# emiliofidalgo/liodom

Hardware: AMD Instinct MI355X
Metric: scans/sec (64×1800 cloud, prev_frames=20) at 1 GPU; pose RMSE vs CPU ref (higher is better)
Workload: dtype f64

## Files before the change

### liodom_amd/csrc/kernels_lm.h

```cpp
__host__ __device__ __forceinline__ bool lm_lds_reduce_fits(int edge_cap) {
  return (size_t)((edge_cap + 3) & ~3) * sizeof(int) + (size_t)kAccN * kLmEvalThreads * sizeof(double) + 8192 <= 160 * 1024;
}
__host__ __device__ __forceinline__ size_t lm_lds_bytes(int edge_cap) {
  return (size_t)((edge_cap + 3) & ~3) * sizeof(int) +
         (lm_lds_reduce_fits(edge_cap) ? (size_t)kAccN * kLmEvalThreads : (size_t)(kLmThreads / 16) * kAccN) * sizeof(double);
}


__device__ int lm_compact_bits(const DevView& v, int s, int outer_it, int E, int* idx ) {
  const int lane = threadIdx.x & 63;
  const int Q = v.knn_queries;
  const int nb = (E + Q - 1) / Q;
  const int nwords = (nb + 3) >> 2;
  const unsigned int* mw = reinterpret_cast<const unsigned int*>(v.corr_mask + ((size_t)s * 2 + outer_it) * v.mask_stride);
  int run = 0;
  for (int w0 = 0; w0 < nwords; w0 += 64) {
    const int w = w0 + lane;
    unsigned int word = (w < nwords) ? mw[w] : 0u;
    const int pop = __popc(word);
    const int incl = wave_incl_scan_i32(pop);
    int o = run + incl - pop;
    while (word) {
      const int b = __ffs(word) - 1;
      word &= word - 1u;
// ... 8 lines not shown
#ifndef LIODOM_LM_CACHED
#define LIODOM_LM_CACHED 1
#endif
constexpr int kLmCached = LIODOM_LM_CACHED;
struct LmCache { float4 P[kLmCached], A[kLmCached], B[kLmCached]; };
__device__ __forceinline__ void lm_cache_load(const DevView& v, int s, int outer_it, int eb, int c_lo, int c_hi, const int* idx, LmCache& k) {
  const float4* ed = v.edges + ((size_t)eb * v.n_streams + s) * v.edge_cap;
  const float4* ca = v.corr_a + ((size_t)s * 2 + outer_it) * v.edge_cap;
  const float4* cb = v.corr_b + ((size_t)s * 2 + outer_it) * v.edge_cap;
  const int et = (int)threadIdx.x;
#pragma unroll
  for (int j = 0; j < kLmCached; j++) {
    const int c = c_lo + et + j * kLmEvalThreads;
    if (et < kLmCtl && c < c_hi) { const int e = idx[c]; k.A[j] = ca[e]; k.B[j] = cb[e]; k.P[j] = ed[e]; }
  }
}

__device__ __forceinline__ void lm_eval(const DevView& v, int s, int outer_it, int eb, int c_lo, int c_hi, const int* idx, const double* Rm_sh,
                                        double* part, double* acc_out , const LmCache& k) {
  const int et = (int)threadIdx.x;
#ifdef LIODOM_LM_NOCACHE
  const bool cached = false;
#else
  const bool cached = et < kLmCtl;
#endif
  double acc[kAccN];
#pragma unroll
  for (int i = 0; i < kAccN; i++) acc[i] = 0.0;
  {
    double Rm[12];
#pragma unroll
    for (int i = 0; i < 12; i++) Rm[i] = Rm_sh[i];
    const float4* ed = v.edges + ((size_t)eb * v.n_streams + s) * v.edge_cap;
    const float4* ca = v.corr_a + ((size_t)s * 2 + outer_it) * v.edge_cap;
    const float4* cb = v.corr_b + ((size_t)s * 2 + outer_it) * v.edge_cap;
    int c = c_lo + et;
    if (cached) {
#pragma unroll
      for (int j = 0; j < kLmCached; j++, c += kLmEvalThreads) {
        if (c < c_hi) {
          const double p[3] = {(double)k.P[j].x, (double)k.P[j].y, (double)k.P[j].z};
          const double a[3] = {(double)k.A[j].x, (double)k.A[j].y, (double)k.A[j].z};
          const double b[3] = {(double)k.B[j].x, (double)k.B[j].y, (double)k.B[j].z};
          residual_accumulate(Rm, p, a, b, v.min_range, v.max_range, acc);
        }
      }
    }
    for (; c < c_hi; c += kLmEvalThreads) {
      const int e = idx[c];
      const float4 A = ca[e];
      const float4 B = cb[e];
      const float4 P = ed[e];
      const double p[3] = {(double)P.x, (double)P.y, (double)P.z};
      const double a[3] = {(double)A.x, (double)A.y, (double)A.z};
      const double b[3] = {(double)B.x, (double)B.y, (double)B.z};
      residual_accumulate(Rm, p, a, b, v.min_range, v.max_range, acc);
    }
  }
  if (v.lm_lds_reduce) {
    const int nb_here = c_hi - c_lo;
    const int ncol = ((nb_here < kLmEvalThreads ? nb_here : kLmEvalThreads) + 15) & ~15;
    if (et < ncol) {
#pragma unroll
      for (int i = 0; i < kAccN; i++) part[i * kLmEvalThreads + et] = acc[i];
    }
    __syncthreads();
    const int r = threadIdx.x & 15;
#pragma unroll
    for (int vrow = threadIdx.x >> 4; vrow < ((kAccN + kLmThreads / 16 - 1) / (kLmThreads / 16)) * (kLmThreads / 16); vrow += kLmThreads / 16) {
      double x = 0.0;
      if (vrow < kAccN) {
        const double* rowp = part + vrow * kLmEvalThreads + r;
        const int nk = ncol >> 4;
#pragma unroll 8
        for (int kk = 0; kk < nk; kk++) x += rowp[kk * 16];
      }
      x = row_sum_f64(x);
      if (vrow < kAccN && r == 0) acc_out[vrow] = x;
    }
    __syncthreads();
    return;
  }
#pragma unroll
  for (int i = 0; i < kAccN; i++) acc[i] = row_sum_f64(acc[i]);
  const int row = threadIdx.x >> 4;
  if ((threadIdx.x & 15) == 0) {
#pragma unroll
    for (int i = 0; i < kAccN; i++) part[row * kAccN + i] = acc[i];
  }
  __syncthreads();
  if (threadIdx.x < kAccN) {
    double x = 0.0;
    for (int w = 0; w < kLmThreads / 16; w++) x += part[w * kAccN + threadIdx.x];
    acc_out[threadIdx.x] = x;
  }
  __syncthreads();
}

__device__ void hash_clear_used(const DevView& v, int s , int nup, int t, int nt) {
  CellSlot empty; empty.key = kEmptyKey; empty.start = 0; empty.cnt = 0;
  const int* used = v.used_cells + (size_t)s * v.used_cap;
  if (nup > v.used_cap) nup = v.used_cap;
  for (int u0 = t; u0 < nup; u0 += 8 * nt) {
    int hh[8];
#pragma unroll
    for (int k = 0; k < 8; k++) { const int u = u0 + k * nt; hh[k] = (u < nup) ? used[u] : -1; }
#pragma unroll
    for (int k = 0; k < 8; k++) {
      if (hh[k] >= 0) {
        const size_t ti = (size_t)s * v.table_size + hh[k];
        v.cells[ti] = empty;
        v.cell_bits[ti >> 5] = 0u;
        if (v.cell_pad) v.cell_pad[ti] = 0u;
      }
    }
  }
}
// ... 159 lines not shown
  if (!st.initialized) return;
  double odom[12], out[12], l2b[12], q[4];
#pragma unroll
  for (int k = 0; k < 12; k++) { odom[k] = st.odom[k]; l2b[k] = v.laser_to_base[k]; }
#pragma unroll
  for (int k = 0; k < 4; k++) q[k] = v.imu_q[(size_t)(s0 + i) * 4 + k];
  imu_override(odom, q, l2b, v.rotation_mode, out);
#pragma unroll
  for (int k = 0; k < 12; k++) st.odom[k] = out[k];
  quat_from_pose(out, v.rotation_mode, st.param_q);
  st.param_t[0] = out[3]; st.param_t[1] = out[7]; st.param_t[2] = out[11];
}

__device__ __forceinline__ void rebuild_beside_solve(const DevView& v, int s, StreamState& st, int eb, int outer_it, int block, int nblocks, unsigned int seq, int* sbase, int* sslot);

template <int kOuterIt, bool kChainMode>
#ifndef LIODOM_LM_WAVES_PER_SIMD
#define LIODOM_LM_WAVES_PER_SIMD 1
#endif
__global__ __launch_bounds__(kLmThreads, LIODOM_LM_WAVES_PER_SIMD) void k_lm_solve(DevView v, int s0, int eb, unsigned int seq, unsigned int done_target) {
  constexpr int outer_it = kOuterIt;
  constexpr int chain = kChainMode ? 1 : 0;
  __shared__ double sh_pose2[2][12];
  __shared__ int sh_pi, sh_ci;
  __shared__ int sh_nmoved;
  __shared__ double sh_pred_s[20];
  __shared__ int sh_unapplied;
  __shared__ double sh_acc[kAccN];
  __shared__ LmState lm;
  __shared__ int sh_flag;
  __shared__ int sh_C;
  const int s = s0 + blockIdx.y;
#if defined(LIODOM_CHAIN_PRIO)
  if (v.n_streams <= 4) __builtin_amdgcn_s_setprio(LIODOM_CHAIN_PRIO);
#endif
  const int G = v.lm_groups, gstride = G > 1 ? 8 : 1, bxl = (int)blockIdx.x;
  const bool is_solver = bxl < G * gstride && (bxl % gstride) == 0;
  const int g = is_solver ? bxl / gstride : G + (bxl < G * gstride ? bxl - (bxl / gstride + 1) : bxl - G);
  StreamState& st = v.state[s];
  __shared__ int sh_cnt[kMaxFrames + 1];
  __shared__ int sh_same_xcc;
  OV_STAMP(v, bxl == 0 && threadIdx.x == 0, outer_it == 0 ? 0 : 3);
  if (seq && outer_it == 0 && bxl == 0 && threadIdx.x == 0) {
    typedef __attribute__((address_space(1))) unsigned int gu32;
    __hip_atomic_store((gu32*)(v.ov_flags + s), seq, __ATOMIC_RELAXED, __HIP_MEMORY_SCOPE_AGENT);
  }
  if (g >= G) {
    if (!v.early_rebuild || chain) return;
    __shared__ int sh_slot[kMaxFrames];
    rebuild_beside_solve(v, s, st, eb, outer_it, g - G, (int)gridDim.x - G, seq, sh_cnt, sh_slot);
    return;
  }
  __shared__ double sh_loc[kAccN];
  __shared__ double sh_red[16][32];
  __shared__ double sh_x0[8];
  __shared__ double sh_prev[12];
  __shared__ int sh_fc;
  if (threadIdx.x < 4) sh_x0[threadIdx.x] = st.param_q[threadIdx.x];
  else if (threadIdx.x < 7) sh_x0[threadIdx.x] = st.param_t[threadIdx.x - 4];
  else if (threadIdx.x >= 64 && threadIdx.x < 76) sh_prev[threadIdx.x - 64] = st.prev_odom[threadIdx.x - 64];
  else if (threadIdx.x == 76) sh_fc = st.frame_count;
  __shared__ int sh_spec_at;
  if (threadIdx.x == 77) sh_spec_at = st.spec_eval[outer_it];
  __shared__ int sh_redo;
  if (threadIdx.x == 78) sh_redo = st.spec_redo[outer_it == 0 ? 1 : 0];
  extern __shared__ __attribute__((aligned(16))) int sh_idx[];
  double* sh_part = reinterpret_cast<double*>(sh_idx + ((v.edge_cap + 3) & ~3));
  const int tid = threadIdx.x;
  const bool prep = tid < kLmCtl;
  bool dead = false;
  if (chain && outer_it == 0) dead = !chain_wait_count(v.knn_done0 + s, done_target, &st.status);
  if (chain && outer_it == 0 && sh_redo) __builtin_amdgcn_fence(__ATOMIC_ACQUIRE, "agent");
  int E_in;
  if (chain && outer_it == 0) {
    typedef __attribute__((address_space(1))) unsigned int gu32;
    E_in = (int)__hip_atomic_load((gu32*)(v.edge_cnt + eb * 32 + s), __ATOMIC_RELAXED, __HIP_MEMORY_SCOPE_AGENT);
  } else {
    E_in = st.n_edges_buf[eb];
  }
  if (outer_it == 0 && tid == 0 && g == 0) {
    st.info.n_edges = E_in;
    st.info.map_points = st.n_search;
    for (int k = 0; k < 2; k++) {
      st.info.lm[k].iterations = 0; st.info.lm[k].accepted = 0; st.info.lm[k].termination = LM_TERM_NO_RESIDUALS;
      st.info.lm[k].pad = 0; st.info.lm[k].initial_cost = 0.0; st.info.lm[k].final_cost = 0.0;
    }
  }
  if (!st.initialized) {
    if (outer_it == 1 && g == 0) {
      if (seq) ov_wait_knn_done(v, s, seq, &st.status);
      if (tid == 0) st.append_raw = 1;
      __shared__ double sh_T0[12];
// ... 49 lines not shown
        for (int u = 0; u < 16; u += 2) { x0 += xs[u]; x1 += xs[u + 1]; }
      }
    }
    sh_red[r0][i] = x0 + x1;
    __syncthreads();
    if (tid <= kAccN) {
      double x = 0.0;
#pragma unroll
      for (int r = 0; r < kRC; r++) x += sh_red[r][tid];
      if (tid < kAccN) sh_acc[tid] = x;
      else { sh_nmatch = (int)x; if (g == 0) st.info.matches[outer_it] = (int)x; }
    }
    __syncthreads();
    nblocks = sh_nmatch;
  } else {
    __syncthreads();
    if (prep) {
      const int C = lm_compact_bits(v, s, outer_it, E, sh_idx);
      if (tid == 0) sh_C = C;
    } else if (tid == kLmCtl) {
      iso_from_qt(sh_x0, sh_x0 + 4, sh_pose2[0]);
    }
    __syncthreads();
    my_share(sh_C);
    lm_cache_load(v, s, outer_it, eb, c_lo, c_hi, sh_idx, cache);
    if (G > 1) { lm_eval(v, s, outer_it, eb, c_lo, c_hi, sh_idx, sh_pose2[0], sh_part, sh_loc, cache); lm_exchange(v, s, g, G, epoch0 | ++n_eval, sh_loc, sh_acc, &st.status, xch_local, &sh_same_xcc); xch_local = sh_same_xcc != 0; }
    else { lm_eval(v, s, outer_it, eb, c_lo, c_hi, sh_idx, sh_pose2[0], sh_part, sh_acc, cache); ++n_eval; }
  }
  DBG_STAMP(v, dbgb, 2, 2);
  int dbg_it = 0;
  int pi = 0, ci = -1, nmoved = 0;
  const unsigned int n_eval0 = n_eval;
  const bool spec_ok = v.speculate != 0 && v.speculate != 5 && v.speculate != 7 && g == 0 && seq != 0u && outer_it == 0;
  const bool spec_ok1 = v.speculate != 0 && v.speculate != 4 && v.speculate != 6 && g == 0 && chain != 0 && outer_it == 1 && v.early_rebuild && v.pred_xch != nullptr;
  const bool spec_forced = v.speculate == 2 || v.speculate == 6 || v.speculate == 7;
  bool spec_done = false;
  int spec_moves = -1;
  for (int step = 0;; step++) {
    if (step == 0 && tid > kLmCtl && tid <= kLmCtl + 6) {
      const int j = tid - kLmCtl - 1;
      sh_scale[j] = 1.0 / (1.0 + sqrt(sh_acc[7 + h_idx(j, j)]));
    }
    if (step == 0) __builtin_amdgcn_wave_barrier();
    if (tid == kLmCtl) {
      const int acc_before = step == 0 ? 0 : lm.accepted;
      const int f = step == 0 ? lm_begin(lm, sh_x0, sh_x0 + 4, sh_acc, nblocks, v.apply_on_ftol, sh_scale) : lm_update(lm, sh_acc);
      sh_flag = f;
      bool moved = step > 0 && lm.accepted != acc_before;
      if (step > 0 && !moved && f != LM_NEED_EVAL && lm.termination == LM_TERM_FUNC_TOL) {
        moved = true;
        for (int k = 0; k < 4; k++) moved = moved && lm.q[k] == lm.cand_q[k];
        for (int k = 0; k < 3; k++) moved = moved && lm.t[k] == lm.cand_t[k];
      }
      if (moved) { ci = pi; pi ^= 1; nmoved++; }
      if (f == LM_NEED_EVAL) iso_from_qt(lm.cand_q, lm.cand_t, sh_pose2[pi]);
      sh_pi = pi; sh_ci = ci; sh_nmoved = nmoved; sh_unapplied = (step > 0 && !moved) ? 1 : 0;
      if (step == 0) DBG_STAMP(v, dbgb, 2, 23);
    } else if (!prep) {
    } else if (step == 0 && v.knn_partials) {
      DBG_STAMP(v, dbge, 2, 24);
      const int C = dead ? 0 : lm_compact_bits(v, s, outer_it, E, sh_idx);
      if (tid == 0) sh_C = C;
      DBG_STAMP(v, dbge, 2, 25);
      my_share(C);
      lm_cache_load(v, s, outer_it, eb, c_lo, c_hi, sh_idx, cache);
    } else if (clr_pending) {
      clear_hash_slots();
    }
    __syncthreads();
    if (step == 0) { if (v.knn_partials && !prep) my_share(sh_C); DBG_STAMP(v, dbgb, 2, 3); }
    else { DBG_STAMP(v, dbgb && dbg_it < 5, 2, 5 + 2 * dbg_it); dbg_it++; }
    if (sh_flag != LM_NEED_EVAL) break;
    if ((spec_ok || spec_ok1) && !spec_done && sh_ci >= 0 &&
        (spec_forced || (!spec_forced && sh_spec_at == 0 && lm.model_cost_change <= v.spec_theta * 1e-6 * lm.cost))) {
      if (spec_ok) {
        ov_publish_pose(v, s, sh_pose2[sh_ci], &lm.q[0], seq, tid, 1);
        OV_STAMP(v, tid == 0, 19);
      } else if (tid >= kLmCtl) {
        const int l = tid - kLmCtl;
        if (l < 25) publish_final_pose(v, s, sh_pose2[sh_ci], 0, (unsigned int)sh_fc + 1u, l, 0);
        if (l == 0) predict_next(sh_pose2[sh_ci], sh_prev, v.rotation_mode, sh_pred_s);
        asm volatile("s_waitcnt lgkmcnt(0)" ::: "memory");
        __builtin_amdgcn_wave_barrier();
        pred_publish(v, s, sh_pred_s, (unsigned int)sh_fc + 1u, l, 64, 1);
        OV_STAMP(v, l == 0, 22);
      }
      if ((kInstrument && (v.debug & 64)) && tid == 0) atomicAdd(&v.dbg_clk[270], 1ull);
      spec_done = true;
      spec_moves = sh_nmoved;
    }
    const double* pose_c = sh_pose2[sh_pi];
    if (G > 1) { lm_eval(v, s, outer_it, eb, c_lo, c_hi, sh_idx, pose_c, sh_part, sh_loc, cache); DBG_STAMP(v, dbgb && dbg_it < 4, 2, 12 + dbg_it); lm_exchange(v, s, g, G, epoch0 | ++n_eval, sh_loc, sh_acc, &st.status, xch_local, &sh_same_xcc); xch_local = sh_same_xcc != 0; }
    else { lm_eval(v, s, outer_it, eb, c_lo, c_hi, sh_idx, pose_c, sh_part, sh_acc, cache); ++n_eval; }
    DBG_STAMP(v, dbgb && dbg_it < 5, 2, 4 + 2 * dbg_it);
  }
  if (clr_pending) clear_hash_slots();
  DBG_STAMP(v, dbgb, 2, 20);
  if ((kInstrument && (v.debug & 32)) && dbgb) v.dbg_clk[2 * 32 + 27] = (xch_local ? 100ull : 0ull) + 10ull * xcc_id() + (unsigned long long)n_eval;
  if (g != 0) return;
  __shared__ double sh_ov[20];
  __shared__ liodom_lm_trace_t sh_trace;
  {
    if (tid == kLmCtl) {
      sh_trace.iterations = lm.iter; sh_trace.accepted = lm.accepted; sh_trace.termination = lm.termination; sh_trace.pad = 0;
      sh_trace.initial_cost = lm.initial_cost; sh_trace.final_cost = lm.cost;
    }
    const int cif = sh_ci;
    if (cif >= 0) {
      if (tid < 12) sh_ov[tid] = sh_pose2[cif][tid];
      else if (tid >= 64 && tid < 71) sh_ov[12 + tid - 64] = (&lm.q[0])[tid - 64];
    } else if (tid == kLmCtl) {
      double q[4], t[3], T[12];
      for (int k = 0; k < 4; k++) q[k] = lm.q[k];
      for (int k = 0; k < 3; k++) t[k] = lm.t[k];
      iso_from_qt(q, t, T);
      for (int k = 0; k < 12; k++) sh_ov[k] = T[k];
      for (int k = 0; k < 4; k++) sh_ov[12 + k] = q[k];
      for (int k = 0; k < 3; k++) sh_ov[16 + k] = t[k];
    }
  }
  __syncthreads();
  if (outer_it == 0) {
    if (seq) { ov_publish_pose(v, s, sh_ov, sh_ov + 12, seq, tid, spec_done ? 2 : 3); OV_STAMP(v, tid == 0, 1); }
  } else if (v.early_rebuild && tid < 50) {
    if (tid >= 25 || !spec_done) publish_final_pose(v, s, sh_ov, 0, (unsigned int)sh_fc + 1u, tid % 25, tid / 25);
  }
  if (tid == kLmCtl) {
    if (outer_it == 0) {
      for (int k = 0; k < 4; k++) st.param_q[k] = sh_ov[12 + k];
      for (int k = 0; k < 3; k++) st.param_t[k] = sh_ov[16 + k];
      for (int k = 0; k < 12; k++) st.odom[k] = sh_ov[k];
    }
    st.spec_eval[outer_it] = (spec_done && sh_nmoved != spec_moves) ? v.spec_backoff : (sh_spec_at > 0 ? sh_spec_at - 1 : 0);
    st.spec_redo[outer_it] = (spec_done && sh_nmoved != spec_moves) ? 1 : 0;
    if (spec_done) { st.spec_stats[2 * outer_it] += 1; if (sh_nmoved != spec_moves) st.spec_stats[2 * outer_it + 1] += 1; }
    if (outer_it == 0) st.info.lm[0] = sh_trace;
    if (outer_it == 1) st.append_raw = 0;
  }
  DBG_STAMP(v, dbgb, 2, 21);
  if (outer_it == 1) {
    finalize_scan(v, s, st, sh_cnt, eb, false, kLmCtl, chain, sh_ov, 0, false, sh_prev, sh_fc, spec_done ? 2 : 3, (!spec_done || sh_nmoved == spec_moves) ? 1u : 2u, &sh_trace);
    DBG_STAMP(v, dbgb, 2, 22);
  }
  DBG_STAMP(v, dbgb, 2, 28);
  OV_STAMP(v, tid == 0, outer_it == 0 ? 2 : 5);
}
```

### liodom_amd/csrc/kernels_sync.h

```cpp
#ifndef LIODOM_POLL_POSE
#define LIODOM_POLL_POSE 6
#endif
#ifndef LIODOM_POLL_DONE
#define LIODOM_POLL_DONE 4
#endif
__device__ __forceinline__ bool pipe_wait(const unsigned int* flag, unsigned int want, unsigned int* status) {
  typedef __attribute__((address_space(1))) unsigned int gu32;
  __shared__ int s_pipe_ok;
  if (threadIdx.x == 0) {
    unsigned int spins = 0;
    unsigned long long t0 = 0;
    bool ok = true;
    while ((int)(__hip_atomic_load((gu32*)flag, __ATOMIC_RELAXED, __HIP_MEMORY_SCOPE_AGENT) - want) < 0) {
      __builtin_amdgcn_s_sleep(8);
      if (++spins > 1500000u || wait_expired(spins, t0)) { atomicOr(status, LIODOM_STATUS_PIPE_TIMEOUT); ok = false; break; }
    }
    if (spins) __builtin_amdgcn_fence(__ATOMIC_ACQUIRE, "agent");
    s_pipe_ok = ok ? 1 : 0;
    INJECT_DELAY(1);
  }
  __syncthreads();
  return s_pipe_ok != 0;
}
__global__ void k_pipe_gate(DevView v, int s0, int eb, unsigned int wait_edges, unsigned int signal_odo) {
  typedef __attribute__((address_space(1))) unsigned int gu32;
  INJECT_DELAY(2);
  if (signal_odo && threadIdx.x == 0) __hip_atomic_store((gu32*)(v.pipe_flags + kEdgePipeBufs), signal_odo, __ATOMIC_RELAXED, __HIP_MEMORY_SCOPE_AGENT);
  if (wait_edges && !pipe_wait(v.pipe_flags + eb, wait_edges, &v.state[s0].status)) {
    for (int s = (int)threadIdx.x; s < v.n_streams; s += (int)blockDim.x) atomicOr(&v.state[s].status, LIODOM_STATUS_PIPE_TIMEOUT);
  }
}
__device__ __forceinline__ void wt_store_u64(void* p, unsigned long long x) {
  typedef __attribute__((address_space(1))) unsigned long long gu64;
  __hip_atomic_store((gu64*)p, x, __ATOMIC_RELAXED, __HIP_MEMORY_SCOPE_AGENT);
}
__device__ __forceinline__ void wt_store_f4(float4* p, const float4& x) {
  wt_store_u64(p, ((unsigned long long)__float_as_uint(x.y) << 32) | __float_as_uint(x.x));
  wt_store_u64(reinterpret_cast<char*>(p) + 8, ((unsigned long long)__float_as_uint(x.w) << 32) | __float_as_uint(x.z));
}
__device__ __forceinline__ void wt_store_u8(void* p, unsigned char x) {
  typedef __attribute__((address_space(1))) unsigned char gu8;
  __hip_atomic_store((gu8*)p, x, __ATOMIC_RELAXED, __HIP_MEMORY_SCOPE_AGENT);
}
constexpr int kOvFinalOffset = 64;
__device__ __forceinline__ void ov_publish_pose(const DevView& v, int s, const double* T, const double* qt, unsigned int tag, int tid, int copies) {
  typedef __attribute__((address_space(1))) unsigned long long gu64;
  const int per = kOvReplicas * kOvGranules;
  INJECT_DELAY(3);
  for (int t = tid; t < 2 * per; t += (int)blockDim.x) {
    const int c = t / per, u = t % per;
    if (!((copies >> c) & 1)) continue;
    const int rep = u / kOvGranules, gi = u % kOvGranules;
    const double val = (gi >> 1) < 12 ? T[gi >> 1] : qt[(gi >> 1) - 12];
    const unsigned long long bits = (unsigned long long)__double_as_longlong(val);
    const unsigned int word = (gi & 1) ? (unsigned int)(bits >> 32) : (unsigned int)bits;
    __hip_atomic_store((gu64*)(v.pose_xch0 + ((size_t)s * kOvReplicas + rep) * 512 + c * kOvFinalOffset + gi), ((unsigned long long)tag << 32) | word,
                       __ATOMIC_RELAXED, __HIP_MEMORY_SCOPE_AGENT);
  }
}
template <int kPollSleep>
__device__ __forceinline__ bool granules_wait(const unsigned long long* base, int n_gran, unsigned int tag, double* out, unsigned int* status) {
  typedef __attribute__((address_space(1))) unsigned long long gu64;
  __shared__ int s_ov_ok;
  const int tid = (int)threadIdx.x;
  if (tid < 64) {
    unsigned long long g = 0, t0 = 0;
    unsigned int spins = 0;
    bool ok;
    while (true) {
      if (tid < n_gran) g = __hip_atomic_load((gu64*)(base + tid), __ATOMIC_RELAXED, __HIP_MEMORY_SCOPE_AGENT);
      ok = tid >= n_gran || (unsigned int)(g >> 32) == tag;
      if (__all(ok)) break;
// ... 196 lines not shown
```

### liodom_amd/csrc/liodom_kernels.h

```cpp
#pragma once
#include <hip/hip_runtime.h>

#include <cstddef>

#include "../../include/liodom_hip.h"
#include "liodom_math.h"
#include "wave_ops.h"

namespace liodom_dev {

#ifndef LIODOM_CHAIN_PRIO
#define LIODOM_CHAIN_PRIO 2
#endif
constexpr int kWave = 64;
constexpr uint64_t kEmptyKey = 0xFFFFFFFFFFFFFFFFull;
#ifndef LIODOM_LM_THREADS
#define LIODOM_LM_THREADS 256
#endif
constexpr int kLmThreads = LIODOM_LM_THREADS;
constexpr int kLmEvalThreads = kLmThreads;
constexpr int kLmCtl = kLmThreads - 64;
#ifndef LIODOM_LM_GROUPS_MAX
#define LIODOM_LM_GROUPS_MAX 8
#endif
constexpr int kLmGroupsMax = LIODOM_LM_GROUPS_MAX;
constexpr int kKnnGroup = 32;
constexpr int kMaxFrames = 256;
constexpr int kEdgeBufs = 4;
constexpr int kEdgePipeBufs = 3;
constexpr int kEdgeBufX = 3;
constexpr int kOvReplicas = 8;
constexpr int kOvGranules = 38;
constexpr int kPredGranules = 38;

struct StreamState {
  double odom[12];
  double prev_odom[12];
  double final_odom[12];
  double param_q[4];
  double param_t[3];
  int32_t initialized;
  int32_t append_raw;
  int32_t frame_count;
  int32_t n_frames;
// ... 233 lines not shown
```

### liodom_amd/csrc/liodom_math.h

```cpp
#pragma once
#include <cfloat>
#include <cmath>
#include <cstdint>

#if defined(__HIPCC__)
#define LD_HD __host__ __device__ __forceinline__
#define LD_UNROLL _Pragma("unroll")
#define LD_FP_CONTRACT_FAST _Pragma("clang fp contract(fast)")
#else
#define LD_HD inline
#define LD_UNROLL
#define LD_FP_CONTRACT_FAST
#endif
#if defined(__HIP_DEVICE_COMPILE__)
#define LD_RSQRT(x) rsqrt(x)
#else
#define LD_RSQRT(x) (1.0 / sqrt(x))
#endif

namespace liodom_dev {

constexpr int kJacobiSweeps = 8;
constexpr int kLmMaxIterations = 4;
constexpr double kHuberA = 0.2;
// ... 243 lines not shown
  const double t_bl[3] = {odom_bl[3], odom_bl[7], odom_bl[11]};
  iso_from_qt(q_new, t_bl, odom_bl);
  iso_inverse(laser_to_base, l2b_inv);
  iso_mul(odom_bl, l2b_inv, out);
}
LD_HD void odom_message(const double* prev_odom, const double* odom, const double* laser_to_base,
                        double delta_time, int rotation_mode, double* out) {
  double bl[12], pbl[12], pinv[12], d[12], qd[4], m[9], roll, pitch, yaw;
  iso_mul(odom, laser_to_base, bl);
  quat_from_pose(bl, rotation_mode, out);
  out[4] = bl[3]; out[5] = bl[7]; out[6] = bl[11];
  iso_mul(prev_odom, laser_to_base, pbl);
  iso_inverse(pbl, pinv);
  iso_mul(pinv, bl, d);
  out[7] = d[3] / delta_time; out[8] = d[7] / delta_time; out[9] = d[11] / delta_time;
  quat_from_pose(d, rotation_mode, qd);
  tf_matrix_from_quat(qd, m);
  tf_get_rpy(m, &roll, &pitch, &yaw);
  out[10] = roll / delta_time; out[11] = pitch / delta_time; out[12] = yaw / delta_time;
}
LD_HD void quat_plus(const double* x, const double* delta, double* out) {
  LD_FP_CONTRACT_FAST
  const double u2 = delta[0] * delta[0] + delta[1] * delta[1] + delta[2] * delta[2];
  if (u2 > 0.0) {
    double s, aw;
    if (u2 < 0.25) {
      const double u = u2;
      s = 1.0 + u * (-1.0 / 6.0 + u * (1.0 / 120.0 + u * (-1.0 / 5040.0 + u * (1.0 / 362880.0 + u * (-1.0 / 39916800.0 +
          u * (1.0 / 6227020800.0 + u * (-1.0 / 1307674368000.0 + u * (1.0 / 355687428096000.0))))))));
      aw = 1.0 + u * (-0.5 + u * (1.0 / 24.0 + u * (-1.0 / 720.0 + u * (1.0 / 40320.0 + u * (-1.0 / 3628800.0 +
           u * (1.0 / 479001600.0 + u * (-1.0 / 87178291200.0 + u * (1.0 / 20922789888000.0))))))));
    } else {
      const double nd = sqrt(u2);
      s = sin(nd) / nd;
      aw = cos(nd);
    }
    const double ax = s * delta[0], ay = s * delta[1], az = s * delta[2];
    const double bw = x[3], bx = x[0], by = x[1], bz = x[2];
    out[3] = aw * bw - ax * bx - ay * by - az * bz;
    out[0] = aw * bx + ax * bw + ay * bz - az * by;
    out[1] = aw * by + ay * bw + az * bx - ax * bz;
    out[2] = aw * bz + az * bw + ax * by - ay * bx;
  } else {
    out[0] = x[0]; out[1] = x[1]; out[2] = x[2]; out[3] = x[3];
  }
}

LD_HD float sqdist_f(float qx, float qy, float qz, float mx, float my, float mz) {
  const float dx = qx - mx, dy = qy - my, dz = qz - mz;
  float r = dx * dx;
  r = r + dy * dy;
  r = r + dz * dz;
  return r;
}

LD_HD void jacobi_rot(double& app, double& aqq, double& apq, double& arp, double& arq) {
  if (fabs(apq) <= 1e-20 * (fabs(app) + fabs(aqq))) return;
  const double theta = (aqq - app) / (2.0 * apq);
  const double at = fabs(theta);
  double t = 1.0 / (at + sqrt(theta * theta + 1.0));
  if (theta < 0.0) t = -t;
  const double c = 1.0 / sqrt(t * t + 1.0);
  const double s = t * c;
  app = app - t * apq;
  aqq = aqq + t * apq;
  apq = 0.0;
  const double nrp = c * arp - s * arq;
  const double nrq = s * arp + c * arq;
// ... 338 lines not shown
    st.cost = cand_cost;
    double gmax = 0.0;
    LD_UNROLL
    for (int j = 0; j < 6; j++) { st.g[j] = acc[1 + j]; const double ag = fabs(st.g[j]); if (ag > gmax) gmax = ag; }
    LD_UNROLL
    for (int j = 0; j < 21; j++) st.H[j] = acc[7 + j];
    st.accepted++;
    const double c = 2.0 * rel - 1.0;
    double f = 1.0 - c * c * c;
    if (f < 1.0 / 3.0) f = 1.0 / 3.0;
    st.radius = st.radius / f;
    if (st.radius > 1e16) st.radius = 1e16;
    st.decrease_factor = 2.0;
    st.reuse_diagonal = 0;
    if (gmax <= 1e-10) { st.termination = LM_TERM_GRAD_TOL; return LM_DONE; }
  } else {
    st.radius = st.radius / st.decrease_factor;
    st.decrease_factor *= 2.0;
    st.reuse_diagonal = 1;
  }
  return lm_propose(st);
}

}
```

Before: 14480.

## Split LM solve into dedicated controller wave overlapping evaluator waves

```diff
diff --git a/liodom_amd/csrc/kernels_lm.h b/liodom_amd/csrc/kernels_lm.h
--- a/liodom_amd/csrc/kernels_lm.h
+++ b/liodom_amd/csrc/kernels_lm.h
@@ -54,20 +54,25 @@
 #ifdef LIODOM_LM_NOCACHE
   const bool cached = false;
 #else
-  const bool cached = et < kLmCtl;
+  const bool cached = true;
 #endif
-  double acc[kAccN];
-#pragma unroll
-  for (int i = 0; i < kAccN; i++) acc[i] = 0.0;
-  {
-    double Rm[12];
-#pragma unroll
-    for (int i = 0; i < 12; i++) Rm[i] = Rm_sh[i];
-    const float4* ed = v.edges + ((size_t)eb * v.n_streams + s) * v.edge_cap;
-    const float4* ca = v.corr_a + ((size_t)s * 2 + outer_it) * v.edge_cap;
-    const float4* cb = v.corr_b + ((size_t)s * 2 + outer_it) * v.edge_cap;
-    int c = c_lo + et;
-    if (cached) {
+  const int nb_here = c_hi - c_lo;
+  const int ncol = ((nb_here < kLmEvalThreads ? nb_here : kLmEvalThreads) + 15) & ~15;
+  const int npass = (et >= kLmCtl - 64 && (!v.lm_lds_reduce || kLmCtl < nb_here)) ? 2 : 1;
+  double Rm[12];
+#pragma unroll
+  for (int i = 0; i < 12; i++) Rm[i] = Rm_sh[i];
+  const float4* ed = v.edges + ((size_t)eb * v.n_streams + s) * v.edge_cap;
+  const float4* ca = v.corr_a + ((size_t)s * 2 + outer_it) * v.edge_cap;
+  const float4* cb = v.corr_b + ((size_t)s * 2 + outer_it) * v.edge_cap;
+#pragma unroll 1
+  for (int pass = 0; pass < npass; pass++) {
+    const int col = et + pass * 64;
+    double acc[kAccN];
+#pragma unroll
+    for (int i = 0; i < kAccN; i++) acc[i] = 0.0;
+    int c = c_lo + col;
+    if (cached && pass == 0) {
 #pragma unroll
       for (int j = 0; j < kLmCached; j++, c += kLmEvalThreads) {
         if (c < c_hi) {
@@ -88,18 +93,26 @@
       const double b[3] = {(double)B.x, (double)B.y, (double)B.z};
       residual_accumulate(Rm, p, a, b, v.min_range, v.max_range, acc);
     }
-  }
+    if (v.lm_lds_reduce) {
+      if (col < ncol) {
+#pragma unroll
+        for (int i = 0; i < kAccN; i++) part[i * kLmEvalThreads + col] = acc[i];
+      }
+    } else {
+#pragma unroll
+      for (int i = 0; i < kAccN; i++) acc[i] = row_sum_f64(acc[i]);
+      if ((col & 15) == 0) {
+#pragma unroll
+        for (int i = 0; i < kAccN; i++) part[(col >> 4) * kAccN + i] = acc[i];
+      }
+    }
+  }
+  __syncthreads();
   if (v.lm_lds_reduce) {
-    const int nb_here = c_hi - c_lo;
-    const int ncol = ((nb_here < kLmEvalThreads ? nb_here : kLmEvalThreads) + 15) & ~15;
-    if (et < ncol) {
-#pragma unroll
-      for (int i = 0; i < kAccN; i++) part[i * kLmEvalThreads + et] = acc[i];
-    }
-    __syncthreads();
-    const int r = threadIdx.x & 15;
-#pragma unroll
-    for (int vrow = threadIdx.x >> 4; vrow < ((kAccN + kLmThreads / 16 - 1) / (kLmThreads / 16)) * (kLmThreads / 16); vrow += kLmThreads / 16) {
+    constexpr int kRows = kLmCtl / 16;
+    const int r = et & 15;
+#pragma unroll
+    for (int vrow = et >> 4; vrow < ((kAccN + kRows - 1) / kRows) * kRows; vrow += kRows) {
       double x = 0.0;
       if (vrow < kAccN) {
         const double* rowp = part + vrow * kLmEvalThreads + r;
@@ -110,21 +123,10 @@
       x = row_sum_f64(x);
       if (vrow < kAccN && r == 0) acc_out[vrow] = x;
     }
-    __syncthreads();
-    return;
-  }
-#pragma unroll
-  for (int i = 0; i < kAccN; i++) acc[i] = row_sum_f64(acc[i]);
-  const int row = threadIdx.x >> 4;
-  if ((threadIdx.x & 15) == 0) {
-#pragma unroll
-    for (int i = 0; i < kAccN; i++) part[row * kAccN + i] = acc[i];
-  }
-  __syncthreads();
-  if (threadIdx.x < kAccN) {
+  } else if (et < kAccN) {
     double x = 0.0;
-    for (int w = 0; w < kLmThreads / 16; w++) x += part[w * kAccN + threadIdx.x];
-    acc_out[threadIdx.x] = x;
+    for (int w = 0; w < kLmThreads / 16; w++) x += part[w * kAccN + et];
+    acc_out[et] = x;
   }
   __syncthreads();
 }
@@ -330,12 +332,13 @@
   constexpr int outer_it = kOuterIt;
   constexpr int chain = kChainMode ? 1 : 0;
   __shared__ double sh_pose2[2][12];
-  __shared__ int sh_pi, sh_ci;
-  __shared__ int sh_nmoved;
+  __shared__ int sh_pi;
   __shared__ double sh_pred_s[20];
-  __shared__ int sh_unapplied;
   __shared__ double sh_acc[kAccN];
-  __shared__ LmState lm;
+  __shared__ double sh_qt[8];
+  __shared__ int sh_spec_done, sh_spec_miss;
+  __shared__ double sh_ov[20];
+  __shared__ liodom_lm_trace_t sh_trace;
   __shared__ int sh_flag;
   __shared__ int sh_C;
   const int s = s0 + blockIdx.y;
@@ -376,6 +379,7 @@
   double* sh_part = reinterpret_cast<double*>(sh_idx + ((v.edge_cap + 3) & ~3));
   const int tid = threadIdx.x;
   const bool prep = tid < kLmCtl;
+  const bool ctl_wave = __builtin_amdgcn_readfirstlane(tid) >= kLmCtl;
   bool dead = false;
   if (chain && outer_it == 0) dead = !chain_wait_count(v.knn_done0 + s, done_target, &st.status);
   if (chain && outer_it == 0 && sh_redo) __builtin_amdgcn_fence(__ATOMIC_ACQUIRE, "agent");
@@ -471,104 +475,133 @@
       iso_from_qt(sh_x0, sh_x0 + 4, sh_pose2[0]);
     }
     __syncthreads();
-    my_share(sh_C);
-    lm_cache_load(v, s, outer_it, eb, c_lo, c_hi, sh_idx, cache);
-    if (G > 1) { lm_eval(v, s, outer_it, eb, c_lo, c_hi, sh_idx, sh_pose2[0], sh_part, sh_loc, cache); lm_exchange(v, s, g, G, epoch0 | ++n_eval, sh_loc, sh_acc, &st.status, xch_local, &sh_same_xcc); xch_local = sh_same_xcc != 0; }
-    else { lm_eval(v, s, outer_it, eb, c_lo, c_hi, sh_idx, sh_pose2[0], sh_part, sh_acc, cache); ++n_eval; }
+    if (!ctl_wave) {
+      my_share(sh_C);
+      lm_cache_load(v, s, outer_it, eb, c_lo, c_hi, sh_idx, cache);
+      if (G > 1) { lm_eval(v, s, outer_it, eb, c_lo, c_hi, sh_idx, sh_pose2[0], sh_part, sh_loc, cache); lm_exchange(v, s, g, G, epoch0 | ++n_eval, sh_loc, sh_acc, &st.status, xch_local, &sh_same_xcc); xch_local = sh_same_xcc != 0; }
+      else { lm_eval(v, s, outer_it, eb, c_lo, c_hi, sh_idx, sh_pose2[0], sh_part, sh_acc, cache); ++n_eval; }
+    } else {
+      __syncthreads(); __syncthreads();
+      if (G > 1) __syncthreads();
+    }
   }
   DBG_STAMP(v, dbgb, 2, 2);
-  int dbg_it = 0;
-  int pi = 0, ci = -1, nmoved = 0;
-  const unsigned int n_eval0 = n_eval;
   const bool spec_ok = v.speculate != 0 && v.speculate != 5 && v.speculate != 7 && g == 0 && seq != 0u && outer_it == 0;
   const bool spec_ok1 = v.speculate != 0 && v.speculate != 4 && v.speculate != 6 && g == 0 && chain != 0 && outer_it == 1 && v.early_rebuild && v.pred_xch != nullptr;
   const bool spec_forced = v.speculate == 2 || v.speculate == 6 || v.speculate == 7;
-  bool spec_done = false;
-  int spec_moves = -1;
-  for (int step = 0;; step++) {
-    if (step == 0 && tid > kLmCtl && tid <= kLmCtl + 6) {
-      const int j = tid - kLmCtl - 1;
+  if (ctl_wave) {
+    const int l = tid - kLmCtl;
+    if (l >= 1 && l <= 6) {
+      const int j = l - 1;
       sh_scale[j] = 1.0 / (1.0 + sqrt(sh_acc[7 + h_idx(j, j)]));
     }
-    if (step == 0) __builtin_amdgcn_wave_barrier();
-    if (tid == kLmCtl) {
-      const int acc_before = step == 0 ? 0 : lm.accepted;
-      const int f = step == 0 ? lm_begin(lm, sh_x0, sh_x0 + 4, sh_acc, nblocks, v.apply_on_ftol, sh_scale) : lm_update(lm, sh_acc);
-      sh_flag = f;
-      bool moved = step > 0 && lm.accepted != acc_before;
-      if (step > 0 && !moved && f != LM_NEED_EVAL && lm.termination == LM_TERM_FUNC_TOL) {
-        moved = true;
-        for (int k = 0; k < 4; k++) moved = moved && lm.q[k] == lm.cand_q[k];
-        for (int k = 0; k < 3; k++) moved = moved && lm.t[k] == lm.cand_t[k];
-      }
-      if (moved) { ci = pi; pi ^= 1; nmoved++; }
-      if (f == LM_NEED_EVAL) iso_from_qt(lm.cand_q, lm.cand_t, sh_pose2[pi]);
-      sh_pi = pi; sh_ci = ci; sh_nmoved = nmoved; sh_unapplied = (step > 0 && !moved) ? 1 : 0;
-      if (step == 0) DBG_STAMP(v, dbgb, 2, 23);
-    } else if (!prep) {
-    } else if (step == 0 && v.knn_partials) {
-      DBG_STAMP(v, dbge, 2, 24);
-      const int C = dead ? 0 : lm_compact_bits(v, s, outer_it, E, sh_idx);
-      if (tid == 0) sh_C = C;
-      DBG_STAMP(v, dbge, 2, 25);
-      my_share(C);
-      lm_cache_load(v, s, outer_it, eb, c_lo, c_hi, sh_idx, cache);
-    } else if (clr_pending) {
-      clear_hash_slots();
-    }
-    __syncthreads();
-    if (step == 0) { if (v.knn_partials && !prep) my_share(sh_C); DBG_STAMP(v, dbgb, 2, 3); }
-    else { DBG_STAMP(v, dbgb && dbg_it < 5, 2, 5 + 2 * dbg_it); dbg_it++; }
-    if (sh_flag != LM_NEED_EVAL) break;
-    if ((spec_ok || spec_ok1) && !spec_done && sh_ci >= 0 &&
-        (spec_forced || (!spec_forced && sh_spec_at == 0 && lm.model_cost_change <= v.spec_theta * 1e-6 * lm.cost))) {
-      if (spec_ok) {
-        ov_publish_pose(v, s, sh_pose2[sh_ci], &lm.q[0], seq, tid, 1);
-        OV_STAMP(v, tid == 0, 19);
-      } else if (tid >= kLmCtl) {
-        const int l = tid - kLmCtl;
-        if (l < 25) publish_final_pose(v, s, sh_pose2[sh_ci], 0, (unsigned int)sh_fc + 1u, l, 0);
-        if (l == 0) predict_next(sh_pose2[sh_ci], sh_prev, v.rotation_mode, sh_pred_s);
+    __builtin_amdgcn_wave_barrier();
+    int pi = 0, ci = -1, nmoved = 0, spec_moves = -1, r = LM_DONE;
+    bool spec_done = false;
+    LmCtl lm;
+    if (l == 0) {
+      const int f = lm_ctl_begin(lm, sh_x0, sh_x0 + 4, sh_acc, nblocks, v.apply_on_ftol, sh_scale);
+      if (f == LM_NEED_EVAL) iso_from_qt(lm.new_q, lm.new_t, sh_pose2[pi]);
+      sh_flag = f; sh_pi = pi;
+      DBG_STAMP(v, dbgb, 2, 23);
+    }
+    for (int step = 0;; step++) {
+      __syncthreads();
+      if (step == 0) DBG_STAMP(v, dbgb, 2, 3);
+      else if (step < 6) DBG_STAMP(v, dbgb, 2, 3 + 2 * step);
+      if (__builtin_amdgcn_readfirstlane(sh_flag) != LM_NEED_EVAL) break;
+      int spec = 0;
+      if (l == 0) {
+        r = lm_ctl_settle(lm);
+        spec = (spec_ok || spec_ok1) && !spec_done && r == LM_NEED_EVAL && ci >= 0 &&
+               (spec_forced || (sh_spec_at == 0 && lm.model_cost_change <= v.spec_theta * 1e-6 * lm.cost));
+        if (spec) {
+          for (int k = 0; k < 4; k++) sh_qt[k] = lm.q[k];
+          for (int k = 0; k < 3; k++) sh_qt[4 + k] = lm.t[k];
+          spec_done = true;
+          spec_moves = nmoved;
+        }
+      }
+      if (__builtin_amdgcn_readfirstlane(spec)) {
         asm volatile("s_waitcnt lgkmcnt(0)" ::: "memory");
         __builtin_amdgcn_wave_barrier();
-        pred_publish(v, s, sh_pred_s, (unsigned int)sh_fc + 1u, l, 64, 1);
-        OV_STAMP(v, l == 0, 22);
-      }
-      if ((kInstrument && (v.debug & 64)) && tid == 0) atomicAdd(&v.dbg_clk[270], 1ull);
-      spec_done = true;
-      spec_moves = sh_nmoved;
-    }
-    const double* pose_c = sh_pose2[sh_pi];
-    if (G > 1) { lm_eval(v, s, outer_it, eb, c_lo, c_hi, sh_idx, pose_c, sh_part, sh_loc, cache); DBG_STAMP(v, dbgb && dbg_it < 4, 2, 12 + dbg_it); lm_exchange(v, s, g, G, epoch0 | ++n_eval, sh_loc, sh_acc, &st.status, xch_local, &sh_same_xcc); xch_local = sh_same_xcc != 0; }
-    else { lm_eval(v, s, outer_it, eb, c_lo, c_hi, sh_idx, pose_c, sh_part, sh_acc, cache); ++n_eval; }
-    DBG_STAMP(v, dbgb && dbg_it < 5, 2, 4 + 2 * dbg_it);
-  }
-  if (clr_pending) clear_hash_slots();
-  DBG_STAMP(v, dbgb, 2, 20);
-  if ((kInstrument && (v.debug & 32)) && dbgb) v.dbg_clk[2 * 32 + 27] = (xch_local ? 100ull : 0ull) + 10ull * xcc_id() + (unsigned long long)n_eval;
-  if (g != 0) return;
-  __shared__ double sh_ov[20];
-  __shared__ liodom_lm_trace_t sh_trace;
-  {
-    if (tid == kLmCtl) {
+        const double* T_it = sh_pose2[__builtin_amdgcn_readfirstlane(ci)];
+        if (spec_ok) {
+          ov_publish_pose(v, s, T_it, sh_qt, seq, l, 1, 64);
+          OV_STAMP(v, l == 0, 19);
+        } else {
+          if (l < 25) publish_final_pose(v, s, T_it, 0, (unsigned int)sh_fc + 1u, l, 0);
+          if (l == 0) predict_next(T_it, sh_prev, v.rotation_mode, sh_pred_s);
+          asm volatile("s_waitcnt lgkmcnt(0)" ::: "memory");
+          __builtin_amdgcn_wave_barrier();
+          pred_publish(v, s, sh_pred_s, (unsigned int)sh_fc + 1u, l, 64, 1);
+          OV_STAMP(v, l == 0, 22);
+        }
+        if ((kInstrument && (v.debug & 64)) && l == 0) atomicAdd(&v.dbg_clk[270], 1ull);
+      }
+      __syncthreads(); __syncthreads();
+      if (G > 1) __syncthreads();
+      if (step < 5) DBG_STAMP(v, dbgb, 2, 4 + 2 * step);
+      if (l == 0) {
+        int f = LM_DONE;
+        if (r == LM_NEED_EVAL) {
+          const int acc_before = lm.accepted;
+          f = lm_ctl_update(lm, sh_acc);
+          bool moved = lm.accepted != acc_before;
+          if (!moved && f != LM_NEED_EVAL && lm.termination == LM_TERM_FUNC_TOL) {
+            moved = true;
+            for (int k = 0; k < 4; k++) moved = moved && lm.q[k] == lm.cand_q[k];
+            for (int k = 0; k < 3; k++) moved = moved && lm.t[k] == lm.cand_t[k];
+          }
+          if (moved) { ci = pi; pi ^= 1; nmoved++; }
+        } else if (r == LM_CTL_RETRY) {
+          f = lm_ctl_form(lm);
+        }
+        if (f == LM_NEED_EVAL) iso_from_qt(lm.new_q, lm.new_t, sh_pose2[pi]);
+        sh_flag = f; sh_pi = pi;
+      }
+    }
+    DBG_STAMP(v, dbgb, 2, 20);
+    const int cif = __builtin_amdgcn_readfirstlane(ci);
+    if (cif >= 0 && l < 12) sh_ov[l] = sh_pose2[cif][l];
+    if (l == 0) {
+      for (int k = 0; k < 4; k++) sh_ov[12 + k] = lm.q[k];
+      for (int k = 0; k < 3; k++) sh_ov[16 + k] = lm.t[k];
+      if (cif < 0) {
+        double q[4], t[3];
+        for (int k = 0; k < 4; k++) q[k] = lm.q[k];
+        for (int k = 0; k < 3; k++) t[k] = lm.t[k];
+        iso_from_qt(q, t, sh_ov);
+      }
       sh_trace.iterations = lm.iter; sh_trace.accepted = lm.accepted; sh_trace.termination = lm.termination; sh_trace.pad = 0;
       sh_trace.initial_cost = lm.initial_cost; sh_trace.final_cost = lm.cost;
-    }
-    const int cif = sh_ci;
-    if (cif >= 0) {
-      if (tid < 12) sh_ov[tid] = sh_pose2[cif][tid];
-      else if (tid >= 64 && tid < 71) sh_ov[12 + tid - 64] = (&lm.q[0])[tid - 64];
-    } else if (tid == kLmCtl) {
-      double q[4], t[3], T[12];
-      for (int k = 0; k < 4; k++) q[k] = lm.q[k];
-      for (int k = 0; k < 3; k++) t[k] = lm.t[k];
-      iso_from_qt(q, t, T);
-      for (int k = 0; k < 12; k++) sh_ov[k] = T[k];
-      for (int k = 0; k < 4; k++) sh_ov[12 + k] = q[k];
-      for (int k = 0; k < 3; k++) sh_ov[16 + k] = t[k];
-    }
-  }
+      sh_spec_done = spec_done ? 1 : 0;
+      sh_spec_miss = (spec_done && nmoved != spec_moves) ? 1 : 0;
+    }
+  } else {
+    for (int step = 0;; step++) {
+      if (step == 0 && v.knn_partials) {
+        DBG_STAMP(v, dbge, 2, 24);
+        const int C = dead ? 0 : lm_compact_bits(v, s, outer_it, E, sh_idx);
+        if (tid == 0) sh_C = C;
+        DBG_STAMP(v, dbge, 2, 25);
+        my_share(C);
+        lm_cache_load(v, s, outer_it, eb, c_lo, c_hi, sh_idx, cache);
+      } else if (clr_pending) {
+        clear_hash_slots();
+      }
+      __syncthreads();
+      if (__builtin_amdgcn_readfirstlane(sh_flag) != LM_NEED_EVAL) break;
+      const double* pose_c = sh_pose2[sh_pi];
+      if (G > 1) { lm_eval(v, s, outer_it, eb, c_lo, c_hi, sh_idx, pose_c, sh_part, sh_loc, cache); DBG_STAMP(v, dbge && step < 4, 2, 12 + step); lm_exchange(v, s, g, G, epoch0 | ++n_eval, sh_loc, sh_acc, &st.status, xch_local, &sh_same_xcc); xch_local = sh_same_xcc != 0; }
+      else { lm_eval(v, s, outer_it, eb, c_lo, c_hi, sh_idx, pose_c, sh_part, sh_acc, cache); ++n_eval; }
+    }
+    if (clr_pending) clear_hash_slots();
+  }
+  if ((kInstrument && (v.debug & 32)) && dbge) v.dbg_clk[2 * 32 + 27] = (xch_local ? 100ull : 0ull) + 10ull * xcc_id() + (unsigned long long)n_eval;
+  if (g != 0) return;
   __syncthreads();
+  const bool spec_done = sh_spec_done != 0, spec_miss = sh_spec_miss != 0;
   if (outer_it == 0) {
     if (seq) { ov_publish_pose(v, s, sh_ov, sh_ov + 12, seq, tid, spec_done ? 2 : 3); OV_STAMP(v, tid == 0, 1); }
   } else if (v.early_rebuild && tid < 50) {
@@ -580,15 +613,15 @@
       for (int k = 0; k < 3; k++) st.param_t[k] = sh_ov[16 + k];
       for (int k = 0; k < 12; k++) st.odom[k] = sh_ov[k];
     }
-    st.spec_eval[outer_it] = (spec_done && sh_nmoved != spec_moves) ? v.spec_backoff : (sh_spec_at > 0 ? sh_spec_at - 1 : 0);
-    st.spec_redo[outer_it] = (spec_done && sh_nmoved != spec_moves) ? 1 : 0;
-    if (spec_done) { st.spec_stats[2 * outer_it] += 1; if (sh_nmoved != spec_moves) st.spec_stats[2 * outer_it + 1] += 1; }
+    st.spec_eval[outer_it] = spec_miss ? v.spec_backoff : (sh_spec_at > 0 ? sh_spec_at - 1 : 0);
+    st.spec_redo[outer_it] = spec_miss ? 1 : 0;
+    if (spec_done) { st.spec_stats[2 * outer_it] += 1; if (spec_miss) st.spec_stats[2 * outer_it + 1] += 1; }
     if (outer_it == 0) st.info.lm[0] = sh_trace;
     if (outer_it == 1) st.append_raw = 0;
   }
   DBG_STAMP(v, dbgb, 2, 21);
   if (outer_it == 1) {
-    finalize_scan(v, s, st, sh_cnt, eb, false, kLmCtl, chain, sh_ov, 0, false, sh_prev, sh_fc, spec_done ? 2 : 3, (!spec_done || sh_nmoved == spec_moves) ? 1u : 2u, &sh_trace);
+    finalize_scan(v, s, st, sh_cnt, eb, false, kLmCtl, chain, sh_ov, 0, false, sh_prev, sh_fc, spec_done ? 2 : 3, spec_miss ? 2u : 1u, &sh_trace);
     DBG_STAMP(v, dbgb, 2, 22);
   }
   DBG_STAMP(v, dbgb, 2, 28);
diff --git a/liodom_amd/csrc/kernels_sync.h b/liodom_amd/csrc/kernels_sync.h
--- a/liodom_amd/csrc/kernels_sync.h
+++ b/liodom_amd/csrc/kernels_sync.h
@@ -43,11 +43,12 @@
   __hip_atomic_store((gu8*)p, x, __ATOMIC_RELAXED, __HIP_MEMORY_SCOPE_AGENT);
 }
 constexpr int kOvFinalOffset = 64;
-__device__ __forceinline__ void ov_publish_pose(const DevView& v, int s, const double* T, const double* qt, unsigned int tag, int tid, int copies) {
+__device__ __forceinline__ void ov_publish_pose(const DevView& v, int s, const double* T, const double* qt, unsigned int tag, int tid, int copies, int nt = 0) {
   typedef __attribute__((address_space(1))) unsigned long long gu64;
   const int per = kOvReplicas * kOvGranules;
   INJECT_DELAY(3);
-  for (int t = tid; t < 2 * per; t += (int)blockDim.x) {
+  const int stride = nt > 0 ? nt : (int)blockDim.x;
+  for (int t = tid; t < 2 * per; t += stride) {
     const int c = t / per, u = t % per;
     if (!((copies >> c) & 1)) continue;
     const int rep = u / kOvGranules, gi = u % kOvGranules;
diff --git a/liodom_amd/csrc/liodom_kernels.h b/liodom_amd/csrc/liodom_kernels.h
--- a/liodom_amd/csrc/liodom_kernels.h
+++ b/liodom_amd/csrc/liodom_kernels.h
@@ -18,8 +18,9 @@
 #define LIODOM_LM_THREADS 256
 #endif
 constexpr int kLmThreads = LIODOM_LM_THREADS;
+constexpr int kLmCtl = kLmThreads - 64;
 constexpr int kLmEvalThreads = kLmThreads;
-constexpr int kLmCtl = kLmThreads - 64;
+static_assert(kLmCtl >= 64 && kLmCtl % 64 == 0, "k_lm_solve: at least one evaluator wave beside the controller's");
 #ifndef LIODOM_LM_GROUPS_MAX
 #define LIODOM_LM_GROUPS_MAX 8
 #endif
diff --git a/liodom_amd/csrc/liodom_math.h b/liodom_amd/csrc/liodom_math.h
--- a/liodom_amd/csrc/liodom_math.h
+++ b/liodom_amd/csrc/liodom_math.h
@@ -289,6 +289,7 @@
 LD_HD void quat_plus(const double* x, const double* delta, double* out) {
   LD_FP_CONTRACT_FAST
   const double u2 = delta[0] * delta[0] + delta[1] * delta[1] + delta[2] * delta[2];
+  double o0 = x[0], o1 = x[1], o2 = x[2], o3 = x[3];
   if (u2 > 0.0) {
     double s, aw;
     if (u2 < 0.25) {
@@ -304,13 +305,12 @@
     }
     const double ax = s * delta[0], ay = s * delta[1], az = s * delta[2];
     const double bw = x[3], bx = x[0], by = x[1], bz = x[2];
-    out[3] = aw * bw - ax * bx - ay * by - az * bz;
-    out[0] = aw * bx + ax * bw + ay * bz - az * by;
-    out[1] = aw * by + ay * bw + az * bx - ax * bz;
-    out[2] = aw * bz + az * bw + ax * by - ay * bx;
-  } else {
-    out[0] = x[0]; out[1] = x[1]; out[2] = x[2]; out[3] = x[3];
-  }
+    o3 = aw * bw - ax * bx - ay * by - az * bz;
+    o0 = aw * bx + ax * bw + ay * bz - az * by;
+    o1 = aw * by + ay * bw + az * bx - ax * bz;
+    o2 = aw * bz + az * bw + ax * by - ay * bx;
+  }
+  out[0] = o0; out[1] = o1; out[2] = o2; out[3] = o3;
 }
 
 LD_HD float sqdist_f(float qx, float qy, float qz, float mx, float my, float mz) {
@@ -695,4 +695,183 @@
   return lm_propose(st);
 }
 
-}
+enum { LM_CTL_RETRY = 2 };
+
+struct LmCtl {
+  double q[4], t[3];
+  double cand_q[4], cand_t[3];
+  double new_q[4], new_t[3];
+  double y[6];
+  double cost;
+  double g[6], H[21];
+  double scale[6];
+  double diag[6];
+  double radius, decrease_factor;
+  double x_norm;
+  double model_cost_change;
+  double initial_cost;
+  int reuse_diagonal;
+  int iter, accepted, invalid_run, termination;
+  int apply_on_ftol;
+};
+
+LD_HD int lm_ctl_form(LmCtl& st) {
+  LD_FP_CONTRACT_FAST
+  while (true) {
+    if (st.iter >= kLmMaxIterations) { st.termination = LM_TERM_MAX_ITER; return LM_DONE; }
+    if (st.radius < 1e-32) { st.termination = LM_TERM_RADIUS; return LM_DONE; }
+    st.iter++;
+    double sc[6], gs[6];
+    LD_UNROLL
+    for (int i = 0; i < 6; i++) { sc[i] = st.scale[i]; gs[i] = sc[i] * st.g[i]; }
+    double A[21];
+    LD_UNROLL
+    for (int i = 0; i < 6; i++) {
+      LD_UNROLL
+      for (int j = 0; j <= i; j++) A[lt_idx(i, j)] = sc[i] * sc[j] * st.H[h_idx(j, i)];
+    }
+    if (!st.reuse_diagonal) {
+      LD_UNROLL
+      for (int j = 0; j < 6; j++) {
+        double d = A[lt_idx(j, j)];
+        if (d < 1e-6) d = 1e-6;
+        if (d > 1e32) d = 1e32;
+        st.diag[j] = d;
+      }
+    }
+    const double inv_radius = 1.0 / st.radius;
+    LD_UNROLL
+    for (int j = 0; j < 6; j++) A[lt_idx(j, j)] += st.diag[j] * inv_radius;
+    double y[6];
+    const bool ok = chol_solve6_packed(A, gs, y);
+    st.reuse_diagonal = 1;
+    if (!ok) {
+      if (++st.invalid_run >= 5) { st.termination = LM_TERM_INVALID_STEPS; return LM_DONE; }
+      st.radius = st.radius * 0.5;
+      continue;
+    }
+    double delta[6];
+    LD_UNROLL
+    for (int j = 0; j < 6; j++) { st.y[j] = y[j]; delta[j] = -y[j] * sc[j]; }
+    quat_plus(st.q, delta, st.new_q);
+    LD_UNROLL
+    for (int k = 0; k < 3; k++) st.new_t[k] = st.t[k] + delta[3 + k];
+    return LM_NEED_EVAL;
+  }
+}
+
+LD_HD int lm_ctl_settle(LmCtl& st) {
+  LD_FP_CONTRACT_FAST
+  st.x_norm = norm7(st.q, st.t);
+  double sc[6], gs[6], step[6];
+  LD_UNROLL
+  for (int i = 0; i < 6; i++) { sc[i] = st.scale[i]; gs[i] = sc[i] * st.g[i]; step[i] = -st.y[i]; }
+  double sg = 0.0, shs = 0.0;
+  LD_UNROLL
+  for (int i = 0; i < 6; i++) {
+    sg += step[i] * gs[i];
+    double row = 0.0;
+    LD_UNROLL
+    for (int j = 0; j < i; j++) row += (sc[i] * sc[j] * st.H[h_idx(j, i)]) * step[j];
+    shs += step[i] * (2.0 * row + (sc[i] * sc[i] * st.H[h_idx(i, i)]) * step[i]);
+  }
+  const double mcc = -sg - 0.5 * shs;
+  if (!(mcc > 0.0)) {
+    if (++st.invalid_run >= 5) { st.termination = LM_TERM_INVALID_STEPS; return LM_DONE; }
+    st.radius = st.radius * 0.5;
+    return LM_CTL_RETRY;
+  }
+  st.invalid_run = 0;
+  st.model_cost_change = mcc;
+  LD_UNROLL
+  for (int k = 0; k < 4; k++) st.cand_q[k] = st.new_q[k];
+  LD_UNROLL
+  for (int k = 0; k < 3; k++) st.cand_t[k] = st.new_t[k];
+  return LM_NEED_EVAL;
+}
+
+LD_HD int lm_ctl_begin(LmCtl& st, const double* q0, const double* t0, const double* acc,
+                       int n_blocks, int apply_on_ftol, const double* pre_scale = nullptr) {
+  LD_UNROLL
+  for (int k = 0; k < 4; k++) st.q[k] = st.cand_q[k] = st.new_q[k] = q0[k];
+  LD_UNROLL
+  for (int k = 0; k < 3; k++) st.t[k] = st.cand_t[k] = st.new_t[k] = t0[k];
+  st.iter = 0; st.accepted = 0; st.invalid_run = 0; st.termination = LM_TERM_MAX_ITER;
+  st.apply_on_ftol = apply_on_ftol;
+  st.cost = 0.0; st.initial_cost = 0.0; st.model_cost_change = 0.0;
+  st.radius = 1e4; st.decrease_factor = 2.0; st.reuse_diagonal = 0;
+  LD_UNROLL
+  for (int j = 0; j < 6; j++) { st.scale[j] = 1.0; st.diag[j] = 0.0; st.g[j] = 0.0; st.y[j] = 0.0; }
+  LD_UNROLL
+  for (int j = 0; j < 21; j++) st.H[j] = 0.0;
+  st.x_norm = norm7(st.q, st.t);
+  if (n_blocks == 0) { st.termination = LM_TERM_NO_RESIDUALS; return LM_DONE; }
+  if (acc[28] != 0.0) { st.termination = LM_TERM_EVAL_FAILURE; return LM_DONE; }
+  st.cost = acc[0]; st.initial_cost = acc[0];
+  double gmax = 0.0;
+  LD_UNROLL
+  for (int j = 0; j < 6; j++) { st.g[j] = acc[1 + j]; const double ag = fabs(st.g[j]); if (ag > gmax) gmax = ag; }
+  LD_UNROLL
+  for (int j = 0; j < 21; j++) st.H[j] = acc[7 + j];
+  LD_UNROLL
+  for (int j = 0; j < 6; j++) st.scale[j] = pre_scale ? pre_scale[j] : 1.0 / (1.0 + sqrt(st.H[h_idx(j, j)]));
+  if (gmax <= 1e-10) { st.termination = LM_TERM_GRAD_TOL; return LM_DONE; }
+  return lm_ctl_form(st);
+}
+
+LD_HD int lm_ctl_update(LmCtl& st, const double* acc) {
+  LD_FP_CONTRACT_FAST
+  const double cand_cost = (acc[28] != 0.0) ? DBL_MAX : acc[0];
+  double dq[4], dt[3];
+  LD_UNROLL
+  for (int k = 0; k < 4; k++) dq[k] = st.q[k] - st.cand_q[k];
+  LD_UNROLL
+  for (int k = 0; k < 3; k++) dt[k] = st.t[k] - st.cand_t[k];
+  const double step_sq = dq[0] * dq[0] + dq[1] * dq[1] + dq[2] * dq[2] + dq[3] * dq[3] + dt[0] * dt[0] + dt[1] * dt[1] + dt[2] * dt[2];
+  const double ptol = 1e-8 * (st.x_norm + 1e-8);
+  const double ptol_sq = ptol * ptol;
+  bool ptol_hit = step_sq <= ptol_sq * (1.0 - 1e-12);
+  if (!ptol_hit && step_sq <= ptol_sq * (1.0 + 1e-12)) ptol_hit = sqrt(step_sq) <= ptol;
+  if (ptol_hit) { st.termination = LM_TERM_PARAM_TOL; return LM_DONE; }
+  const double cost_change = st.cost - cand_cost;
+  if (fabs(cost_change) <= 1e-6 * st.cost) {
+    st.termination = LM_TERM_FUNC_TOL;
+    if (st.apply_on_ftol && cost_change > 0.0) {
+      LD_UNROLL
+      for (int k = 0; k < 4; k++) st.q[k] = st.cand_q[k];
+      LD_UNROLL
+      for (int k = 0; k < 3; k++) st.t[k] = st.cand_t[k];
+      st.cost = cand_cost;
+    }
+    return LM_DONE;
+  }
+  const double rel = cost_change / st.model_cost_change;
+  if (rel > 1e-3) {
+    LD_UNROLL
+    for (int k = 0; k < 4; k++) st.q[k] = st.cand_q[k];
+    LD_UNROLL
+    for (int k = 0; k < 3; k++) st.t[k] = st.cand_t[k];
+    st.cost = cand_cost;
+    double gmax = 0.0;
+    LD_UNROLL
+    for (int j = 0; j < 6; j++) { st.g[j] = acc[1 + j]; const double ag = fabs(st.g[j]); if (ag > gmax) gmax = ag; }
+    LD_UNROLL
+    for (int j = 0; j < 21; j++) st.H[j] = acc[7 + j];
+    st.accepted++;
+    const double c = 2.0 * rel - 1.0;
+    double f = 1.0 - c * c * c;
+    if (f < 1.0 / 3.0) f = 1.0 / 3.0;
+    st.radius = st.radius / f;
+    if (st.radius > 1e16) st.radius = 1e16;
+    st.decrease_factor = 2.0;
+    st.reuse_diagonal = 0;
+    if (gmax <= 1e-10) { st.termination = LM_TERM_GRAD_TOL; return LM_DONE; }
+  } else {
+    st.radius = st.radius / st.decrease_factor;
+    st.decrease_factor *= 2.0;
+    st.reuse_diagonal = 1;
+  }
+  return lm_ctl_form(st);
+}
+
+}
```

Result: no change. 14580, median of 6 (+0.6%).
